# rrwick/Autocycler

Hardware: NVIDIA H100
Metric: input-assembly Mbp/sec through compress->unitig GFA (higher is better)
Workload: dtype u64

## Files before the change

### autocycler_b200/csrc/pipeline.cu

```cuda
#include "pipeline.h"

#include <algorithm>
#include <cmath>
#include <vector>

unsigned long long g_ac_kernel_launches = 0;

#define AC_NONE32 0xFFFFFFFFu
#define AC_CHUNK 32
#define AC_MINCHUNK 128
#define AC_MAX_RANKS 16
#define AC_BOUND_STRIPES 64
#ifndef AC_INSERT_CTAS
#define AC_INSERT_CTAS 2
#endif

struct TableView {
    Slot* slots;
    uint64_t cap;
    const uint64_t* packed;
    const SeqInfo* seqs;
    uint32_t n_seqs;
    uint32_t* count_big;
    uint32_t gb;
// ... 531 lines not shown
};

struct RunAssignBody {
    const uint64_t* run_start; const uint32_t* run_len; const uint32_t* run_uk; const uint8_t* run_dir;
    const uint32_t* uid_rep; const uint32_t* rep_idx; const uint32_t* run_hs; const uint32_t* run_ts; TableView t;
    uint32_t* run_unitig; DeviceUnitig* unitigs; uint32_t* slot_unitig;
    AC_D void operator()(uint64_t r) const {
        const uint32_t rep = uid_rep[run_uk[r]];
        const uint32_t j = rep_idx[rep];
        run_unitig[r] = (j << 1) | (run_dir[r] == run_dir[rep] ? 1u : 0u);
        if (rep == (uint32_t)r) {
            const uint32_t hs = run_hs[r], ts = run_ts[r];
            DeviceUnitig u;
            u.start = run_start[r]; u.len = run_len[r]; u.depth = table_depth(t, hs); u.flip = 0; u.min_d = 0;
            u.head_slot = hs; u.tail_slot = ts;
            for (int w = 0; w < AC_MAX_W; ++w) u.min_w[w] = 0;
            unitigs[j] = u;
            slot_unitig[hs] = j; slot_unitig[ts] = j;
        }
    }
};

struct ClaimedCountBody { const uint32_t* bits; uint64_t n_words; uint32_t* cnt; AC_D void operator()(uint64_t w) const { cnt[w] = w < n_words ? ac_popc(bits[w]) : 0u; } };
template <int W> struct ClaimedListBody {
    const uint32_t* bits; const uint32_t* off; const uint32_t* pos_slot; uint32_t* list;
    TableView t; KParams p; const uint8_t* interior; uint64_t* filter; uint64_t n_fwords;
    AC_D void operator()(uint64_t g) const {
        const uint32_t m = bits[g >> 5], b = (uint32_t)g & 31u;
        if (!((m >> b) & 1u)) return;
        list[off[g >> 5] + ac_popc(m & ((1u << b) - 1u))] = pos_slot[g];
        if (filter) {
            const Key<W> f = window_key<W>(t, g, !interior[g >> 5], p);
            ext_add_kmer<W>(filter, n_fwords, f, key_rc(f, p), p);
        }
    }
};
struct ExportScatterBody {
    TableView t; const uint32_t* occupied; SlotRec* out;
    AC_D void operator()(uint64_t x) const { const uint64_t i = occupied[x]; SlotRec r; r.slot = t.slots[i]; r.count = table_depth(t, i); r.pad = 0; out[x] = r; }
};
template <int W> struct MergeBody {
    TableView t; KParams p; const SlotRec* in; uint32_t* pos_slot; unsigned long long* counters; uint32_t* claimed_bits;
    AC_D void operator()(uint64_t i) const {
        const SlotRec r = in[i];
        const uint64_t g = slot_gpos(r.slot, t.gb);
        const bool dotted = slot_dotted(r.slot, t.gb);
        const uint32_t flags = slot_flags(r.slot);
        const Key<W> fwd = window_key<W>(t, g, dotted, p);
        const Key<W> rc = key_rc(fwd, p);
        const uint64_t h = key_hash(key_is_canonical(fwd, p) ? fwd : rc);
        const uint32_t tag = make_tag(dotted, h, t.gb);
        const Slot mine = make_slot(g, tag, t.count_big ? 0u : r.count, flags, t.gb);
        if (!t.count_big && r.count >= t.alarm) counters[3] = 1;
        uint64_t slot = table_home(t, h);
        for (uint32_t probes = 0;; ++probes) {
            if (probes > 8192) { counters[2] = 1; return; }
            Slot e = ac_ld_cg(&t.slots[slot]);
            if (e == AC_EMPTY_SLOT) {
                e = ac_atomic_cas(&t.slots[slot], (Slot)AC_EMPTY_SLOT, mine);
                if (e == AC_EMPTY_SLOT) { if (t.count_big) ac_atomic_add(&t.count_big[slot], r.count); if (dotted) ac_atomic_add(&counters[1], 1ull); ac_atomic_or(&claimed_bits[g >> 5], 1u << (g & 31u)); break; }
            }
            if (slot_tag(e, t.gb) == tag) {
                const Key<W> rep = window_key<W>(t, slot_gpos(e, t.gb), dotted, p);
                if (key_eq(rep, fwd) || key_eq(rep, rc)) { slot_add_occurrence(t, slot, e, g, r.count, flags, true, counters); break; }
            }
            if (++slot == t.cap) slot = 0;
        }
        pos_slot[g] = (uint32_t)slot;
    }
};

struct ChunkCountBody {
    const DeviceUnitig* unitigs; uint32_t* nchunks;
    AC_D void operator()(uint64_t j) const { nchunks[j] = (unitigs[j].len + AC_MINCHUNK - 1) / AC_MINCHUNK; }
};

template <int W> struct MinPartial { Key<W> key; uint32_t from_rc; };

template <int W> struct ChunkMinBody {
    const uint64_t* packed; const SeqInfo* seqs; uint32_t n_seqs; KParams p;
    const DeviceUnitig* unitigs; uint32_t n_unitigs; const uint32_t* chunk_off; MinPartial<W>* partial;
    AC_D void operator()(uint64_t c) const {
        uint32_t lo = 0, hi = n_unitigs;
        while (hi - lo > 1) { uint32_t mid = (lo + hi) >> 1; if (chunk_off[mid] <= c) lo = mid; else hi = mid; }
        const DeviceUnitig u = unitigs[lo];
        const uint64_t first = (c - chunk_off[lo]) * AC_MINCHUNK;
        const uint64_t n = (u.len - first < AC_MINCHUNK) ? u.len - first : AC_MINCHUNK;
        uint64_t g = u.start + first;
        const SeqInfo s = seqs[find_seq(seqs, n_seqs, g)];
        uint64_t fs = g - s.start;
        Key<W> fwd, rc, best = Key<W>(); bool rolling = false, have = false; uint32_t best_rc = 0;
        for (uint64_t t = 0; t < n; ++t, ++g, ++fs) {
            const int32_t d = window_dots(s, fs, p.k);
            if (d != 0) { fwd = fetch_codes<W>(packed, g, p); fwd.d = d; rc = key_rc(fwd, p); rolling = false; }
            else if (!rolling) { fwd = fetch_codes<W>(packed, g, p); rc = key_rc(fwd, p); rolling = true; }
            else { const uint64_t code = packed_base(packed, g + p.k - 1); key_push_right(fwd, code, p); key_push_left(rc, 3 - code, p); }
            if (!have || key_less5(fwd, best)) { best = fwd; best_rc = 0; have = true; }
            if (key_less5(rc, best)) { best = rc; best_rc = 1; }
        }
        MinPartial<W> out; out.key = best; out.from_rc = best_rc;
        partial[c] = out;
    }
};

template <int W> struct UnitigMinBody {
    const uint32_t* chunk_off; const MinPartial<W>* partial; DeviceUnitig* unitigs;
    AC_D void operator()(uint64_t j) const {
        const uint32_t c0 = chunk_off[j], c1 = chunk_off[j + 1];
        MinPartial<W> best = partial[c0];
        for (uint32_t c = c0 + 1; c < c1; ++c) { const MinPartial<W> q = partial[c]; if (key_less5(q.key, best.key)) best = q; }
        DeviceUnitig u = unitigs[j];
        u.flip = best.from_rc; u.min_d = best.key.d;
        for (int w = 0; w < W; ++w) u.min_w[w] = best.key.w[w];
        unitigs[j] = u;
    }
};

template <int W> struct LinkBody {
    TableView t; KParams p; bool any_dotted;
    const DeviceUnitig* unitigs; const uint32_t* pos_slot; const uint32_t* slot_unitig;
    uint32_t* link_count; uint32_t* links;
    AC_D void operator()(uint64_t i) const {
        const uint32_t j = (uint32_t)(i >> 1), e = (uint32_t)(i & 1);
        const DeviceUnitig u = unitigs[j];
        Key<W> tail, tail_rc;
        if (e == 0) {
            const uint64_t g = u.start + u.len - 1;
            tail = fetch_codes<W>(t.packed, g, p);
            const SeqInfo s = t.seqs[find_seq(t.seqs, t.n_seqs, g)];
            tail.d = window_dots(s, g - s.start, p.k);
            tail_rc = key_rc(tail, p);
        } else {
            const uint64_t g = u.start;
            tail_rc = fetch_codes<W>(t.packed, g, p);
            const SeqInfo s = t.seqs[find_seq(t.seqs, t.n_seqs, g)];
            tail_rc.d = window_dots(s, g - s.start, p.k);
            tail = key_rc(tail_rc, p);
        }
        uint32_t n = 0;
        for_each_successor<W>(tail, tail_rc, any_dotted, p, [&](const Key<W>& a, const Key<W>& arc) {
            const uint32_t s2 = table_find<W>(t, a, arc, p);
            if (s2 == AC_NONE32) return;
            const uint32_t j2 = slot_unitig[s2];
            const DeviceUnitig v = unitigs[j2];
            const bool a_canon = key_is_canonical(a, p);
            const bool head_fwd = v.head_slot == s2 && ((packed_base(t.packed, v.start + p.h) < 2) == a_canon);
            if (n < AC_MAX_LINKS) links[i * AC_MAX_LINKS + n] = (j2 << 1) | (head_fwd ? 0u : 1u);
            ++n;
        });
        link_count[i] = n;
    }
};

struct alignas(16) SortRec { uint64_t a, b; uint32_t c, d, id, pad; };
struct SeedLess {
    const DeviceUnitig* unitigs; int W;
    typedef SortRec Key;
    AC_D Key load(uint32_t id) const {
        const DeviceUnitig& x = unitigs[id];
        Key k; k.id = id; k.pad = 0; k.a = x.min_w[0]; k.b = W > 1 ? x.min_w[1] : 0; k.c = x.min_d > 0 ? (uint32_t)x.min_d : 0u; k.d = x.min_d < 0 ? (uint32_t)-x.min_d : 0u;
        return k;
    }
    AC_D bool less_keys(const Key& x, const Key& y, uint32_t ia, uint32_t ib) const {
        if (x.c != y.c) return x.c > y.c;
        if (x.a != y.a) return x.a < y.a;
        if (x.b != y.b) return x.b < y.b;
        if (W > 2) return (*this)(ia, ib);
        return x.d > y.d;
    }
    AC_D bool operator()(uint32_t a, uint32_t b) const {
        const DeviceUnitig& x = unitigs[a]; const DeviceUnitig& y = unitigs[b];
        const int lx = x.min_d > 0 ? x.min_d : 0, ly = y.min_d > 0 ? y.min_d : 0;
        if (lx != ly) return lx > ly;
        for (int w = 0; w < W; ++w) if (x.min_w[w] != y.min_w[w]) return x.min_w[w] < y.min_w[w];
        const int tx = x.min_d < 0 ? -x.min_d : 0, ty = y.min_d < 0 ? -y.min_d : 0;
        return tx > ty;
    }
};
#define AC_SORT_LEAF 8
#define AC_SORT_WAYS 8
template <class Less> struct MergeWaysBody {
    Less less; uint32_t n, width, steps; const SortRec* in; SortRec* out; uint32_t* idx_out;
    AC_D void operator()(uint64_t i) const {
        const SortRec me = in[i];
        const uint64_t run = i / width, group = run / AC_SORT_WAYS, group_start = group * AC_SORT_WAYS * (uint64_t)width;
        uint32_t lo[AC_SORT_WAYS], hi[AC_SORT_WAYS];
#pragma unroll
        for (int s = 0; s < AC_SORT_WAYS; ++s) {
            const uint64_t first = group_start + (uint64_t)s * width, last = first + width;
            lo[s] = (uint32_t)(first < n ? first : n); hi[s] = (uint32_t)(last < n ? last : n);
            if (group * AC_SORT_WAYS + s == run) hi[s] = lo[s];
        }
        for (uint32_t step = 0; step < steps; ++step) {
#pragma unroll
            for (int s = 0; s < AC_SORT_WAYS; ++s) {
                if (lo[s] < hi[s]) {
                    const uint32_t mid = (lo[s] + hi[s]) >> 1;
                    const SortRec x = in[mid];
                    const bool earlier = group * AC_SORT_WAYS + s < run;
                    const bool before = earlier ? !less.less_keys(me, x, me.id, x.id) : less.less_keys(x, me, x.id, me.id);
                    if (before) lo[s] = mid + 1; else hi[s] = mid;
                }
            }
        }
        uint64_t pos = group_start + (i - run * width);
#pragma unroll
        for (int s = 0; s < AC_SORT_WAYS; ++s) {
            const uint64_t first = group_start + (uint64_t)s * width;
            if (group * AC_SORT_WAYS + s != run && first < n) pos += lo[s] - (uint32_t)first;
        }
        out[pos] = me; idx_out[pos] = me.id;
    }
};

#ifndef AC_EMULATE
#define AC_SORT_TILE 2048
#else
#define AC_SORT_TILE 16
#endif
#ifndef AC_EMULATE
template <class Less> __global__ void __launch_bounds__(1024) ac_tile_sort_kernel(const Less less, uint32_t n, uint32_t* __restrict__ idx, SortRec* __restrict__ recs) {
    extern __shared__ __align__(16) unsigned char tile_smem[];
    SortRec* keys = reinterpret_cast<SortRec*>(tile_smem);
    uint16_t* buf0 = reinterpret_cast<uint16_t*>(tile_smem + AC_SORT_TILE * sizeof(SortRec));
    uint16_t* buf1 = buf0 + AC_SORT_TILE;
    const uint32_t base = blockIdx.x * AC_SORT_TILE, count = n - base < AC_SORT_TILE ? n - base : AC_SORT_TILE;
    for (uint32_t i = threadIdx.x; i < count; i += blockDim.x) { SortRec r = less.load(base + i); r.id = base + i; r.pad = 0; keys[i] = r; }
    __syncthreads();
    auto before = [&](uint32_t x, uint32_t y) { return less.less_keys(keys[x], keys[y], base + x, base + y); };
    if (threadIdx.x < AC_SORT_TILE / AC_SORT_LEAF) {
        const uint32_t a = threadIdx.x * AC_SORT_LEAF, b = a + AC_SORT_LEAF < count ? a + AC_SORT_LEAF : count;
        uint16_t v[AC_SORT_LEAF];
        for (uint32_t x = a; x < b; ++x) {
            uint32_t y = x - a;
            while (y > 0 && before(x, v[y - 1])) { v[y] = v[y - 1]; --y; }
            v[y] = (uint16_t)x;
        }
        for (uint32_t x = a; x < b; ++x) buf0[x] = v[x - a];
    }
    __syncthreads();
    uint16_t* in = buf0; uint16_t* out = buf1;
    for (uint32_t width = AC_SORT_LEAF; width < count; width *= 2) {
        for (uint32_t i = threadIdx.x; i < count; i += blockDim.x) {
            const uint32_t me = in[i];
            const uint32_t run = i / width, pair_start = (run & ~1u) * width, run_start = run * width;
            const bool left = !(run & 1u);
            uint32_t lo, hi;
            if (left) { lo = run_start + width; hi = lo + width; } else { lo = pair_start; hi = run_start; }
            if (lo > count) lo = count;
            if (hi > count) hi = count;
            const uint32_t first = lo;
            while (lo < hi) { const uint32_t mid = (lo + hi) >> 1; const bool bf = left ? before(in[mid], me) : !before(me, in[mid]); if (bf) lo = mid + 1; else hi = mid; }
            out[pair_start + (i - run_start) + (lo - first)] = (uint16_t)me;
        }
        __syncthreads();
        uint16_t* t = in; in = out; out = t;
    }
    for (uint32_t i = threadIdx.x; i < count; i += blockDim.x) { const SortRec r = keys[in[i]]; recs[base + i] = r; idx[base + i] = r.id; }
}
#endif
template <class Less> struct TileSortBody {
    Less less; uint32_t n; uint32_t* idx; SortRec* recs;
    AC_D void operator()(uint64_t c) const {
        const uint32_t a = (uint32_t)c * AC_SORT_TILE, b = a + AC_SORT_TILE < n ? a + AC_SORT_TILE : n;
        for (uint32_t x = a; x < b; ++x) {
            uint32_t y = x;
            while (y > a && less(x, idx[y - 1])) { idx[y] = idx[y - 1]; --y; }
            idx[y] = x;
        }
        for (uint32_t x = a; x < b; ++x) { SortRec r = less.load(idx[x]); r.id = idx[x]; r.pad = 0; recs[x] = r; }
    }
};
template <class Less> static uint32_t* sort_indices(AcStream* stream, const Less& less, uint32_t n, uint32_t* a, uint32_t* b, SortRec* ra, SortRec* rb) {
    if (n == 0) return a;
    const uint64_t tiles = ((uint64_t)n + AC_SORT_TILE - 1) / AC_SORT_TILE;
#ifndef AC_EMULATE
    const size_t smem = AC_SORT_TILE * (sizeof(SortRec) + 2 * sizeof(uint16_t));
    ac_launch_kernel("tile_sort", stream, ac_tile_sort_kernel<Less>, (unsigned)tiles, 1024, smem, less, n, a, ra);
#else
    ac_launch("tile_sort", stream, TileSortBody<Less>{less, n, a, ra}, tiles);
#endif
    for (uint64_t width = AC_SORT_TILE; width < n; width *= AC_SORT_WAYS) {
        uint32_t steps = 1; while ((1ull << steps) <= width) ++steps;
        ac_launch("merge_pass", stream, MergeWaysBody<Less>{less, n, (uint32_t)width, steps, ra, rb, b}, n);
        std::swap(a, b); std::swap(ra, rb);
    }
    return a;
}

struct NumberKeyBody {
    const UnitigRec* rec; const char* arena; uint64_t* prefix;
    AC_D void operator()(uint64_t s) const {
        const unsigned char* q = (const unsigned char*)(arena + rec[s].seq_off);
        const uint32_t m = rec[s].len < 8 ? rec[s].len : 8;
        uint64_t v = 0;
        for (uint32_t i = 0; i < m; ++i) v |= (uint64_t)q[i] << (56 - 8 * i);
        prefix[s] = v;
    }
};
struct InversePermBody { const uint32_t* order; uint32_t* pos; AC_D void operator()(uint64_t n) const { pos[order[n]] = (uint32_t)n; } };
struct NumberLess {
    const UnitigRec* rec; const uint32_t* depth; const char* arena; const uint64_t* prefix;
    const uint32_t* pos;
    typedef SortRec Key;
    AC_D Key load(uint32_t id) const { Key k; k.id = id; k.pad = 0; k.a = prefix[id]; k.b = pos ? pos[id] : id; k.c = rec[id].len; k.d = depth[id]; return k; }
    AC_D bool less_keys(const Key& x, const Key& y, uint32_t ia, uint32_t ib) const {
        if (x.c != y.c) return x.c > y.c;
        if (x.a != y.a) return x.a < y.a;
        if (x.c > 8) return (*this)(ia, ib);
        if (x.d != y.d) return x.d > y.d;
        return x.b < y.b;
    }
    AC_D bool operator()(uint32_t a, uint32_t b) const {
        const uint32_t la = rec[a].len, lb = rec[b].len;
        if (la != lb) return la > lb;
        if (prefix[a] != prefix[b]) return prefix[a] < prefix[b];
        const char* x = arena + rec[a].seq_off; const char* y = arena + rec[b].seq_off;
        for (uint32_t i = 8; i < la; ++i) if (x[i] != y[i]) return (unsigned char)x[i] < (unsigned char)y[i];
        if (depth[a] != depth[b]) return depth[a] > depth[b];
        return pos ? pos[a] < pos[b] : a < b;
    }
};


struct SeedGatherBody {
    const uint32_t* perm; const DeviceUnitig* unitigs; uint32_t n;
    uint32_t* rank; uint32_t* len; uint32_t* depth; uint32_t* need; uint32_t* min_fpos; uint32_t* min_rpos;
    AC_D void operator()(uint64_t s) const {
        if (s == n) { need[s] = 0; return; }
        const uint32_t j = perm[s];
        const DeviceUnitig& u = unitigs[j];
        rank[j] = (uint32_t)s; len[s] = u.len; depth[s] = u.depth; need[s] = u.len + 2 * AC_SEQ_SLACK;
        min_fpos[s] = 0xFFFFFFFFu; min_rpos[s] = 0xFFFFFFFFu;
    }
};
struct SeqOffBody { const uint32_t* need_off; uint64_t* seq_off; AC_D void operator()(uint64_t s) const { seq_off[s] = (uint64_t)need_off[s] + AC_SEQ_SLACK; } };

struct EmitSeqBody {
    const uint64_t* packed; uint32_t h; const DeviceUnitig* unitigs; uint32_t n_unitigs; const uint32_t* chunk_off;
    const uint32_t* rank; const uint64_t* seq_off; char* arena;
    AC_D void operator()(uint64_t c) const {
        uint32_t lo = 0, hi = n_unitigs;
        while (hi - lo > 1) { uint32_t mid = (lo + hi) >> 1; if (chunk_off[mid] <= c) lo = mid; else hi = mid; }
        const DeviceUnitig u = unitigs[lo];
        const uint64_t first = (c - chunk_off[lo]) * AC_MINCHUNK;
        const uint64_t n = (u.len - first < AC_MINCHUNK) ? u.len - first : AC_MINCHUNK;
        char* dst = arena + seq_off[rank[lo]];
        const uint64_t g0 = u.start + h + first;
        if (!u.flip) for (uint64_t t = 0; t < n; ++t) dst[first + t] = "ACGT"[packed_base(packed, g0 + t)];
        else for (uint64_t t = 0; t < n; ++t) dst[u.len - 1 - (first + t)] = "TGCA"[packed_base(packed, g0 + t)];
    }
};

AC_D UStrand seed_strand(uint32_t dev_strand, const uint32_t* rank, const DeviceUnitig* unitigs) {
    const uint32_t j = dev_strand >> 1;
    return (rank[j] << 1) | ((dev_strand & 1u) ^ (unitigs[j].flip & 1u));
}

struct LinkCountBody {
    const uint32_t* link_count; const uint32_t* rank; const DeviceUnitig* unitigs; uint32_t n_strands; uint32_t* cnt;
    AC_D void operator()(uint64_t i) const {
        if (i == n_strands) { cnt[i] = 0; return; }
        cnt[seed_strand((uint32_t)i, rank, unitigs)] = link_count[i];
    }
};

struct LinkOrderBody {
    const uint32_t* link_count; const uint32_t* links; const uint32_t* rank; const DeviceUnitig* unitigs;
    const uint32_t* next_off; UStrand* next; uint32_t* prev_cnt; uint32_t* hairpins;
    AC_D static uint64_t order_key(UStrand from, UStrand t) {
        const uint32_t a = from >> 1, b = t >> 1; const bool trev = t & 1;
        uint32_t phase;
        if (!(from & 1)) phase = trev ? 1 : 0;
        else phase = trev ? (b < a ? 0 : (b == a ? 1 : 3)) : 2;
        return ((uint64_t)phase << 32) | b;
    }
    AC_D void operator()(uint64_t i) const {
        const UStrand from = seed_strand((uint32_t)i, rank, unitigs);
        const uint32_t n = link_count[i];
        UStrand t[AC_MAX_LINKS];
        for (uint32_t x = 0; x < n && x < AC_MAX_LINKS; ++x) t[x] = seed_strand(links[i * AC_MAX_LINKS + x], rank, unitigs);
        for (uint32_t x = 1; x < n; ++x) {
            const UStrand v = t[x]; const uint64_t kv = order_key(from, v); uint32_t y = x;
            while (y > 0 && order_key(from, t[y - 1]) > kv) { t[y] = t[y - 1]; --y; }
            t[y] = v;
        }
        UStrand* out = next + next_off[from];
        for (uint32_t x = 0; x < n; ++x) { out[x] = t[x]; ac_atomic_add(&prev_cnt[t[x]], 1u); if (t[x] == (from ^ 1u)) ac_atomic_add(hairpins, 1u); }
    }
};
struct PrevFillBody {
    const uint32_t* next_off; const UStrand* next; const uint32_t* prev_off; uint32_t* cursor; UStrand* prev;
    AC_D void operator()(uint64_t from) const {
        for (uint32_t x = next_off[from]; x < next_off[from + 1]; ++x) { const UStrand t = next[x]; prev[prev_off[t] + ac_atomic_add(&cursor[t], 1u)] = (UStrand)from; }
    }
};
struct PrevSortBody {
    const uint32_t* prev_off; UStrand* prev;
    AC_D void operator()(uint64_t s) const {
        UStrand* p = prev + prev_off[s]; const uint32_t n = prev_off[s + 1] - prev_off[s];
        for (uint32_t x = 1; x < n; ++x) { const UStrand v = p[x]; uint32_t y = x; while (y > 0 && p[y - 1] > v) { p[y] = p[y - 1]; --y; } p[y] = v; }
    }
};

struct PathBody {
    const SeqInfo* seqs; uint32_t n_seqs; const uint64_t* run_start; const uint32_t* run_len; const uint32_t* run_unitig;
    const uint32_t* rank; const DeviceUnitig* unitigs; UStrand* path; uint32_t* min_fpos; uint32_t* min_rpos;
    AC_D void operator()(uint64_t x) const {
        const uint32_t dev = run_unitig[x] >> 1, same = run_unitig[x] & 1;
        const uint32_t s = rank[dev];
        const bool plus = (same ^ (unitigs[dev].flip & 1u)) != 0;
        path[x] = (s << 1) | (plus ? 0u : 1u);
        const uint64_t g = run_start[x];
        const SeqInfo q = seqs[find_seq(seqs, n_seqs, g)];
        const uint32_t fs = (uint32_t)(g - q.start), mirrored = q.len - fs - run_len[x];
        ac_atomic_min(&min_fpos[s], plus ? fs : mirrored);
        ac_atomic_min(&min_rpos[s], plus ? mirrored : fs);
    }
};
struct PackRecBody {
    const uint64_t* seq_off; const uint32_t* len; const uint32_t* min_fpos; const uint32_t* min_rpos; UnitigRec* rec;
    AC_D void operator()(uint64_t s) const {
        UnitigRec r; r.seq_off = seq_off[s]; r.len = len[s]; r.min_fpos = min_fpos[s]; r.min_rpos = min_rpos[s];
        r.room_before = AC_SEQ_SLACK; r.room_after = AC_SEQ_SLACK; r.flags = 0;
        rec[s] = r;
    }
};
struct FixedSeedBody {
    const uint64_t* path_off; const UStrand* path; uint8_t* fixed_start; uint8_t* fixed_end;
    AC_D void operator()(uint64_t i) const {
        if (path_off[i + 1] == path_off[i]) return;
        const UStrand first = path[path_off[i]], last = path[path_off[i + 1] - 1];
        if (!(first & 1u)) fixed_start[first >> 1] = 1; else fixed_end[first >> 1] = 1;
        if (!(last & 1u)) fixed_end[last >> 1] = 1; else fixed_start[last >> 1] = 1;
    }
};
struct FixedSpreadBody {
    const uint8_t* seed_start; const uint8_t* seed_end; const uint32_t* next_off; const UStrand* next; const uint32_t* prev_off; const UStrand* prev;
    uint8_t* fixed_start; uint8_t* fixed_end;
    AC_D void operator()(uint64_t u) const {
        const uint32_t s = (uint32_t)u << 1;
        if (seed_start[u]) for (uint32_t x = prev_off[s]; x < prev_off[s + 1]; ++x) { const UStrand up = prev[x]; if (!(up & 1u)) fixed_end[up >> 1] = 1; else fixed_start[up >> 1] = 1; }
        if (seed_end[u]) for (uint32_t x = next_off[s]; x < next_off[s + 1]; ++x) { const UStrand down = next[x]; if (!(down & 1u)) fixed_start[down >> 1] = 1; else fixed_end[down >> 1] = 1; }
    }
};
struct CandidateView {
    const uint32_t* order; const uint32_t* next_off; const UStrand* next; const uint32_t* prev_off; const UStrand* prev;
    const uint8_t* fixed_start; const uint8_t* fixed_end;
    AC_D bool eligible(uint32_t idx, uint32_t side) const {
        const UStrand self = idx << 1;
        const uint32_t* off = side == 0 ? prev_off : next_off; const UStrand* lst = side == 0 ? prev : next;
        const uint32_t* back_off = side == 0 ? next_off : prev_off; const UStrand* back = side == 0 ? next : prev;
        const uint32_t gn = off[self + 1] - off[self];
        if (gn < 2 || (side == 0 ? fixed_start[idx] : fixed_end[idx])) return false;
        for (uint32_t a = 0; a < gn; ++a) {
            const UStrand p = lst[off[self] + a];
            if (back_off[p + 1] - back_off[p] != 1 || back[back_off[p]] != self || (p >> 1) == idx) return false;
            const bool rev = p & 1u;
            if (side == 0 ? ((!rev && fixed_end[p >> 1]) || (rev && fixed_start[p >> 1])) : ((!rev && fixed_start[p >> 1]) || (rev && fixed_end[p >> 1]))) return false;
        }
        return true;
    }
};
struct CandidateFlagBody {
    CandidateView v; uint32_t n; uint32_t* flag;
    AC_D void operator()(uint64_t x) const {
        if (x == 2ull * n) { flag[x] = 0; return; }
        flag[x] = v.eligible(v.order[x >> 1], (uint32_t)(x & 1)) ? 1u : 0u;
    }
};
struct CandidateFillBody {
// ... 883 lines not shown
    }
    any_dotted = n_dotted != 0;
    const TableView tv = table_view();

    flags8.ensure(cap);
    n_slots_used = list_claimed<W>(true);
    const AdjacencyBody<W> adj{tv, p, any_dotted, occ_list.as<uint32_t>(), flags8.as<uint8_t>(), ext_filter.as<uint64_t>(), n_fwords};
    if (is_multi && exp_valid && exp_n + 64 < n_slots_used) {
        const uint64_t n_cw = (total + 31) / 32, n_adj = exp_n + 64;
        if (getenv("AC_HOST_PROFILE")) fprintf(stderr, "[device] adjacency flags for this rank's own k-mers: at most %llu of %llu\n", (unsigned long long)n_adj, (unsigned long long)n_slots_used);
        ac_launch("adjacency", &stream, AdjacencyOwnBody<W>{adj, claimed_cnt.as<uint32_t>(), g_begin >> 5, std::min<uint64_t>((g_end + 31) >> 5, n_cw)}, n_adj);
    } else ac_launch("adjacency", &stream, adj, n_slots_used);
    mark(ADJACENCY_END);

    const uint64_t n_bwords = (total + 31) / 32;
    bmask.ensure(n_bwords * sizeof(uint32_t)); bcount.ensure(n_bwords * sizeof(uint32_t)); boff.ensure(n_bwords * sizeof(uint32_t));
    ac_launch("boundaries", &stream, BoundaryBody{packed.as<uint64_t>(), seqs.as<SeqInfo>(), n_seqs, p.h, g_begin, g_end, pos_slot.as<uint32_t>(),
                                                  flags8.as<uint8_t>(), interior8.as<uint8_t>(), bmask.as<uint32_t>(), bcount.as<uint32_t>()}, n_bwords * 32);
    n_runs = scan(&stream, bcount.as<uint32_t>(), boff.as<uint32_t>(), n_bwords);
    mark(BOUNDARIES_END);
    run_start.ensure(n_runs * sizeof(uint64_t)); run_len.ensure(n_runs * 4); run_hs.ensure(n_runs * 4); run_ts.ensure(n_runs * 4);
    ac_launch("run_scatter", &stream, RunScatterBody{bmask.as<uint32_t>(), boff.as<uint32_t>(), run_start.as<uint64_t>()}, n_bwords);
    ac_launch("run_ends", &stream, RunEndsLocalBody{seqs.as<SeqInfo>(), n_seqs, run_start.as<uint64_t>(), n_runs, pos_slot.as<uint32_t>(),
                                                    run_len.as<uint32_t>(), run_hs.as<uint32_t>(), run_ts.as<uint32_t>()}, n_runs);
    n_own_runs = n_runs;
    stage = Stage::RUNS;
}

void DevicePipeline::export_runs(void* dst, uint64_t cap_records) {
    Impl& m = *impl; m.make_current();
    m.require(Stage::RUNS, "runs_local must precede export_runs");
    if (cap_records < m.n_runs) throw std::runtime_error("run buffer too small");
    ac_launch("run_export", &m.stream, RunExportBody{m.run_start.as<uint64_t>(), m.run_len.as<uint32_t>(), m.run_hs.as<uint32_t>(), m.run_ts.as<uint32_t>(),
                                                     m.slots.as<Slot>(), slot_gpos_bits(m.total), (RunRec*)dst}, m.n_runs);
    ac_sync(&m.stream);
}

void DevicePipeline::import_runs(const void* dev_ptr, uint64_t n) {
    Impl& m = *impl; m.make_current();
    m.require(Stage::RUNS, "runs_local must precede import_runs");
    m.n_runs = n;
    m.run_start.ensure(n * sizeof(uint64_t)); m.run_len.ensure(n * 4); m.run_hs.ensure(n * 4); m.run_ts.ensure(n * 4);
    RunImportBody body{(const RunRec*)dev_ptr, m.pos_slot.as<uint32_t>(), m.run_start.as<uint64_t>(), m.run_len.as<uint32_t>(), m.run_hs.as<uint32_t>(), m.run_ts.as<uint32_t>(), 0, {0}, {nullptr}};
    ac_launch("run_import", &m.stream, body, n);
}

void DevicePipeline::import_runs_from(const void* const* ptrs, const uint64_t* counts, uint32_t n_ranks) {
    Impl& m = *impl; m.make_current();
    m.require(Stage::RUNS, "runs_local must precede import_runs");
    if (n_ranks == 0 || n_ranks > AC_MAX_RANKS) throw std::runtime_error("import_runs: bad rank count");
    RunImportBody body{nullptr, m.pos_slot.as<uint32_t>(), nullptr, nullptr, nullptr, nullptr, n_ranks, {0}, {nullptr}};
    for (uint32_t q = 0; q < n_ranks; ++q) { body.first[q + 1] = body.first[q] + counts[q]; body.src[q] = (const RunRec*)ptrs[q]; }
    const uint64_t n = m.n_runs = body.first[n_ranks];
    m.run_start.ensure(n * sizeof(uint64_t)); m.run_len.ensure(n * 4); m.run_hs.ensure(n * 4); m.run_ts.ensure(n * 4);
    body.run_start = m.run_start.as<uint64_t>(); body.run_len = m.run_len.as<uint32_t>(); body.run_hs = m.run_hs.as<uint32_t>(); body.run_ts = m.run_ts.as<uint32_t>();
    ac_launch("run_import", &m.stream, body, n);
}

void DevicePipeline::finish(PipelineResult& out, bool keep_positions, bool fused, bool split_paths) {
    Impl& m = *impl; m.make_current(); const int W = m.W;
    if (split_paths && !fused) throw std::runtime_error("split path lines need the fused finish");
    AC_DISPATCH_W(m.unitigs_w, out)
    m.host_arrays();
    m.paths();
    m.work_list();
    if (fused && m.R.n_cands > 0) m.simplify();
    m.mark(SIMPLIFY_END);
    if (fused) {
        m.renumber();
        if (m.U < 100000000u) m.gfa(split_paths);
    }
    m.mark(GFA_END);
    m.results(out, keep_positions, fused);
}

template <int W> void DevicePipeline::Impl::unitigs_w(PipelineResult& out) {
    require(Stage::RUNS, "runs_local must precede finish");
    const KParams p = make_kparams(k, W);
    const TableView tv = table_view();
    out = PipelineResult();
    out.W = W; out.capacity = cap; out.n_slots_used = n_slots_used; out.n_dotted = n_dotted;
    R = Pending();
    mark(FINISH_BEGIN);
    run_uk.ensure(n_runs * 4); run_dir.ensure(n_runs);
    is_rep.ensure(n_runs * 4); rep_idx.ensure(n_runs * 4); run_unitig.ensure(n_runs * 4);
    uid_rep.ensure(cap * 4); slot_unitig.ensure(cap * 4);
    ac_memset(uid_rep.p, 0xFF, cap * 4, &stream);
    ac_launch("run_key", &stream, RunKeyBody{packed.as<uint64_t>(), p.h, run_start.as<uint64_t>(), run_hs.as<uint32_t>(), run_ts.as<uint32_t>(),
                                             run_uk.as<uint32_t>(), run_dir.as<uint8_t>(), uid_rep.as<uint32_t>()}, n_runs);
    ac_launch("rep_flag", &stream, RepFlagBody{run_uk.as<uint32_t>(), uid_rep.as<uint32_t>(), is_rep.as<uint32_t>()}, n_runs);
    U = scan(&stream, is_rep.as<uint32_t>(), rep_idx.as<uint32_t>(), n_runs);
    unitigs.ensure((size_t)U * sizeof(DeviceUnitig));
    ac_launch("run_assign", &stream, RunAssignBody{run_start.as<uint64_t>(), run_len.as<uint32_t>(), run_uk.as<uint32_t>(), run_dir.as<uint8_t>(),
                                                   uid_rep.as<uint32_t>(), rep_idx.as<uint32_t>(), run_hs.as<uint32_t>(), run_ts.as<uint32_t>(), tv,
                                                   run_unitig.as<uint32_t>(), unitigs.as<DeviceUnitig>(), slot_unitig.as<uint32_t>()}, n_runs);
    mark(UNITIGS_END);

    nchunks.ensure(((size_t)U + 1) * 4); chunk_off.ensure(((size_t)U + 1) * 4);
    ac_launch("chunk_count", &stream, ChunkCountBody{unitigs.as<DeviceUnitig>(), nchunks.as<uint32_t>()}, U);
    ac_memset(nchunks.as<uint32_t>() + U, 0, 4, &stream);
    n_chunks = scan(&stream, nchunks.as<uint32_t>(), chunk_off.as<uint32_t>(), (uint64_t)U + 1);
    partial.ensure((size_t)n_chunks * sizeof(MinPartial<W>));
    ac_launch("chunk_min", &stream, ChunkMinBody<W>{packed.as<uint64_t>(), seqs.as<SeqInfo>(), n_seqs, p, unitigs.as<DeviceUnitig>(), U,
                                                    chunk_off.as<uint32_t>(), partial.as<MinPartial<W>>()}, n_chunks);
    ac_launch("unitig_min", &stream, UnitigMinBody<W>{chunk_off.as<uint32_t>(), partial.as<MinPartial<W>>(), unitigs.as<DeviceUnitig>()}, U);
    mark(SEEDS_END);

    link_count.ensure((size_t)U * 2 * 4); links.ensure((size_t)U * 2 * AC_MAX_LINKS * 4);
    ac_launch("links", &stream, LinkBody<W>{tv, p, any_dotted, unitigs.as<DeviceUnitig>(), pos_slot.as<uint32_t>(), slot_unitig.as<uint32_t>(),
                                            link_count.as<uint32_t>(), links.as<uint32_t>()}, (uint64_t)U * 2);
    mark(LINKS_END);
}

void DevicePipeline::Impl::host_arrays() {
    sort_a.ensure((size_t)U * 4); sort_b.ensure((size_t)U * 4); sort_ra.ensure((size_t)U * sizeof(SortRec)); sort_rb.ensure((size_t)U * sizeof(SortRec));
    const SeedLess seed_less{unitigs.as<DeviceUnitig>(), W};
    const uint32_t* perm = sort_indices(&stream, seed_less, U, sort_a.as<uint32_t>(), sort_b.as<uint32_t>(), sort_ra.as<SortRec>(), sort_rb.as<SortRec>());
    mark(SEED_SORT_END);
    rank.ensure((size_t)U * 4); d_len.ensure((size_t)U * 4); d_depth.ensure((size_t)U * 4); need.ensure(((size_t)U + 1) * 4);
    d_seq_off.ensure((size_t)U * 8); d_min_fpos.ensure((size_t)U * 4); d_min_rpos.ensure((size_t)U * 4);
    ac_launch("seed_gather", &stream, SeedGatherBody{perm, unitigs.as<DeviceUnitig>(), U, rank.as<uint32_t>(), d_len.as<uint32_t>(), d_depth.as<uint32_t>(),
                                                     need.as<uint32_t>(), d_min_fpos.as<uint32_t>(), d_min_rpos.as<uint32_t>()}, (uint64_t)U + 1);
    if (n_windows + (uint64_t)U * 2 * AC_SEQ_SLACK >= 0xFFFFFFF0ull) throw std::runtime_error("unitig sequence arena would exceed 4 GB");
    const uint64_t arena_bytes = scan(&stream, need.as<uint32_t>(), need.as<uint32_t>(), (uint64_t)U + 1);
    ac_launch("seq_off", &stream, SeqOffBody{need.as<uint32_t>(), d_seq_off.as<uint64_t>()}, U);
    d_arena.ensure(arena_bytes);
    ac_launch("emit_seq", &stream, EmitSeqBody{packed.as<uint64_t>(), make_kparams(k, W).h, unitigs.as<DeviceUnitig>(), U, chunk_off.as<uint32_t>(), rank.as<uint32_t>(),
                                               d_seq_off.as<uint64_t>(), d_arena.as<char>()}, n_chunks);
    R.arena_final = arena_bytes; R.arena_src = &d_arena;
    const uint32_t n_strands = 2 * U;
    strand_cnt.ensure(((size_t)n_strands + 1) * 4); d_next_off.ensure(((size_t)n_strands + 1) * 4);
    prev_cnt.ensure(((size_t)n_strands + 1) * 4); d_prev_off.ensure(((size_t)n_strands + 1) * 4);
    ac_launch("link_count", &stream, LinkCountBody{link_count.as<uint32_t>(), rank.as<uint32_t>(), unitigs.as<DeviceUnitig>(), n_strands, strand_cnt.as<uint32_t>()},
              (uint64_t)n_strands + 1);
    const uint64_t n_links = R.n_links = scan(&stream, strand_cnt.as<uint32_t>(), d_next_off.as<uint32_t>(), (uint64_t)n_strands + 1);
    d_next.ensure(n_links * 4); d_prev.ensure(n_links * 4);
    ac_memset(prev_cnt.p, 0, ((size_t)n_strands + 1) * 4, &stream);
    d_small.ensure(64); ac_memset(d_small.p, 0, 64, &stream);
    ac_launch("link_order", &stream, LinkOrderBody{link_count.as<uint32_t>(), links.as<uint32_t>(), rank.as<uint32_t>(), unitigs.as<DeviceUnitig>(),
                                                   d_next_off.as<uint32_t>(), d_next.as<UStrand>(), prev_cnt.as<uint32_t>(), d_small.as<uint32_t>()}, n_strands);
    scan(&stream, prev_cnt.as<uint32_t>(), d_prev_off.as<uint32_t>(), (uint64_t)n_strands + 1, false);
    ac_memset(prev_cnt.p, 0, ((size_t)n_strands + 1) * 4, &stream);
    ac_launch("prev_fill", &stream, PrevFillBody{d_next_off.as<uint32_t>(), d_next.as<UStrand>(), d_prev_off.as<uint32_t>(), prev_cnt.as<uint32_t>(), d_prev.as<UStrand>()}, n_strands);
    ac_launch("prev_sort", &stream, PrevSortBody{d_prev_off.as<uint32_t>(), d_prev.as<UStrand>()}, n_strands);
}

void DevicePipeline::Impl::paths() {
    d_path.ensure(n_runs * 4); d_path_off.ensure(((size_t)n_seqs + 1) * 8);
    ac_launch("path", &stream, PathBody{seqs.as<SeqInfo>(), n_seqs, run_start.as<uint64_t>(), run_len.as<uint32_t>(), run_unitig.as<uint32_t>(), rank.as<uint32_t>(),
                                        unitigs.as<DeviceUnitig>(), d_path.as<UStrand>(), d_min_fpos.as<uint32_t>(), d_min_rpos.as<uint32_t>()}, n_runs);
    d_rec.ensure((size_t)U * sizeof(UnitigRec));
    ac_launch("pack_rec", &stream, PackRecBody{d_seq_off.as<uint64_t>(), d_len.as<uint32_t>(), d_min_fpos.as<uint32_t>(), d_min_rpos.as<uint32_t>(), d_rec.as<UnitigRec>()}, U);
    ac_launch("path_off", &stream, PathOffBody{seqs.as<SeqInfo>(), n_seqs, run_start.as<uint64_t>(), n_runs, d_path_off.as<uint64_t>()}, (uint64_t)n_seqs + 1);
    num_prefix.ensure((size_t)U * 8);
    ac_launch("number_key", &stream, NumberKeyBody{d_rec.as<UnitigRec>(), d_arena.as<char>(), num_prefix.as<uint64_t>()}, U);
    const NumberLess number_less{d_rec.as<UnitigRec>(), d_depth.as<uint32_t>(), d_arena.as<char>(), num_prefix.as<uint64_t>(), nullptr};
    R.order_built = sort_indices(&stream, number_less, U, sort_a.as<uint32_t>(), sort_b.as<uint32_t>(), sort_ra.as<SortRec>(), sort_rb.as<SortRec>());
}

void DevicePipeline::Impl::work_list() {
    d_fixed.ensure((size_t)U * 4); ac_memset(d_fixed.p, 0, (size_t)U * 4, &stream);
    uint8_t* seed_start = d_fixed.as<uint8_t>(); uint8_t* seed_end = seed_start + U; uint8_t* fix_start = R.fix_start = seed_end + U; uint8_t* fix_end = fix_start + U;
    ac_launch("fixed_seed", &stream, FixedSeedBody{d_path_off.as<uint64_t>(), d_path.as<UStrand>(), seed_start, seed_end}, n_seqs);
    ac_copy_dd(fix_start, seed_start, (size_t)U * 2, &stream);
    ac_launch("fixed_spread", &stream, FixedSpreadBody{seed_start, seed_end, d_next_off.as<uint32_t>(), d_next.as<UStrand>(), d_prev_off.as<uint32_t>(), d_prev.as<UStrand>(),
                                                       fix_start, fix_end}, U);
    const CandidateView cview{R.order_built, d_next_off.as<uint32_t>(), d_next.as<UStrand>(), d_prev_off.as<uint32_t>(), d_prev.as<UStrand>(), fix_start, fix_end};
    cand_flag.ensure((2 * (size_t)U + 1) * 4); cand_index.ensure((2 * (size_t)U + 1) * 4);
    ac_launch("candidate_flag", &stream, CandidateFlagBody{cview, U, cand_flag.as<uint32_t>()}, 2ull * U + 1);
    const uint64_t n_cands = R.n_cands = scan(&stream, cand_flag.as<uint32_t>(), cand_index.as<uint32_t>(), 2ull * U + 1);
    d_cands.ensure((n_cands + 1) * sizeof(ExpandCandidate)); d_cand_at.ensure(2 * (size_t)U * 4 + 4); d_deps.ensure((size_t)U * sizeof(ExpandDeps) + 4); d_spec.ensure((n_cands + 1) * 4);
    ac_launch("candidate_fill", &stream, CandidateFillBody{cview, cand_flag.as<uint32_t>(), cand_index.as<uint32_t>(), d_cands.as<ExpandCandidate>(), d_cand_at.as<int32_t>()}, 2ull * U);
    ac_launch("dependents", &stream, DependentsBody{d_next_off.as<uint32_t>(), d_next.as<UStrand>(), d_prev_off.as<uint32_t>(), d_prev.as<UStrand>(), d_cand_at.as<int32_t>(),
                                                    d_deps.as<ExpandDeps>()}, U);
    ac_launch("common_length", &stream, CommonLengthBody{d_cands.as<ExpandCandidate>(), d_rec.as<UnitigRec>(), d_arena.as<char>(), d_spec.as<uint32_t>()}, n_cands);
    mark(WORK_LIST_END);
}

void DevicePipeline::Impl::simplify() {
    const uint64_t n_cands = R.n_cands, arena_bytes = R.arena_final;
    d_pred.ensure(n_cands * 7 * 4); d_level.ensure(n_cands * 4); d_flagmax.ensure(32); d_counters64.ensure((AC_PASS_WORDS + 8) * 8);
    d_dirty.ensure(((n_cands + 63) / 64) * 8 + 8); d_exhausted.ensure(n_cands + 8);
    unsigned long long* c64 = d_counters64.as<unsigned long long>();
    unsigned long long* res = c64 + AC_PASS_WORDS;
    ac_launch("level_pred", &stream, LevelPredBody{d_cands.as<ExpandCandidate>(), d_deps.as<ExpandDeps>(), d_pred.as<int32_t>()}, n_cands);
    ac_memset(d_level.p, 0, n_cands * 4, &stream); ac_memset(d_flagmax.p, 0, 32, &stream);
    ac_launch_coop("levels", &stream, LevelsCoopBody{d_pred.as<int32_t>(), d_level.as<uint32_t>(), d_flagmax.as<uint32_t>(), n_cands}, n_cands, 1024);
    ac_memset(d_counters64.p, 0, (AC_PASS_WORDS + 8) * 8, &stream);
    const RelocBoundBody bound_body{d_cands.as<ExpandCandidate>(), d_rec.as<UnitigRec>(), d_cand_at.as<int32_t>(), c64 + AC_PASS_SET(1) + 1};
    ac_launch("reloc_bound", &stream, bound_body, n_cands);
    uint32_t fm[8]; unsigned long long h64[AC_PASS_WORDS + 8];
    ac_d2h(fm, d_flagmax.p, 32, &stream); ac_d2h(h64, c64, sizeof h64, &stream); ac_sync(&stream);
    if (fm[4]) throw std::runtime_error("candidate levels did not settle");
    unsigned long long bound = 0; for (int x = 0; x < AC_BOUND_STRIPES; ++x) bound += h64[AC_PASS_SET(1) + 1 + x];
    if (arena_bytes + bound >= 0xFFFFFFF0ull) throw std::runtime_error("unitig sequence arena would exceed 4 GB");
    d_arena2.ensure(arena_bytes + 2 * bound + 64);
    ac_copy_dd(d_arena2.p, d_arena.p, arena_bytes, &stream);
    const unsigned long long start = arena_bytes;
    ac_h2d(c64, &start, 8, &stream);
    ac_memset(c64 + AC_PASS_SET(1), 0, AC_PASS_SET_WORDS * 8, &stream);
    ac_memset(d_dirty.p, 0, ((n_cands + 63) / 64) * 8 + 8, &stream); ac_memset(d_exhausted.p, 0, n_cands + 8, &stream);
    static const bool always_grow = getenv("AC_DEVICE_TIGHT_ARENA") != nullptr;
    uint32_t next_set = 0, next_due = 0; uint64_t passes = 0;
    const uint32_t due_stride = fm[3] + 2;
    d_due.ensure((size_t)3 * due_stride * 4); ac_memset(d_due.p, 0, (size_t)3 * due_stride * 4, &stream);
    for (bool first = true;; first = false) {
        const ApplyLevelBody apply{d_cands.as<ExpandCandidate>(), d_deps.as<ExpandDeps>(), d_level.as<uint32_t>(), 0, d_spec.as<uint32_t>(),
                                   d_rec.as<UnitigRec>(), d_arena2.as<char>(), c64, c64, d_dirty.as<uint64_t>(), d_exhausted.as<uint8_t>(), first, c64 + AC_PASS_REMOVED};
        const uint64_t room = always_grow ? 0 : d_arena2.cap;
        ac_launch_coop("simplify", &stream, SimplifyCoopBody{apply, bound_body, n_cands, d_flagmax.as<uint32_t>() + 3, c64, res, room, next_set, first,
                                                             d_due.as<uint32_t>(), due_stride, next_due}, n_cands, 64);
        ac_d2h(h64, c64, sizeof h64, &stream); ac_sync(&stream);
        const unsigned long long* r = h64 + AC_PASS_WORDS;
        R.arena_final = h64[0]; R.bases_removed = h64[AC_PASS_REMOVED]; R.any_moved = r[1] != 0;
        passes += r[2]; next_set = (uint32_t)r[5]; next_due = (uint32_t)r[7];
        if (getenv("AC_HOST_PROFILE")) fprintf(stderr, "[device] expand_repeats launch: %llu passes (%llu so far), %u levels, %llu candidates, %llu left on the work list, last pass moved %llu bases\n",
                                               r[2], (unsigned long long)passes, fm[3], (unsigned long long)n_cands, r[4], r[0]);
        if (r[0] == 0) break;
        if (passes > 1000000) throw std::runtime_error("repeat expansion did not settle");
        bound = r[3];
        if (R.arena_final + bound >= 0xFFFFFFF0ull) throw std::runtime_error("unitig sequence arena would exceed 4 GB");
        d_arena3.ensure(std::max<size_t>((R.arena_final + bound) * 2 + 64, d_arena3.cap + (always_grow ? 64 : 0)));
        ac_copy_dd(d_arena3.p, d_arena2.p, R.arena_final, &stream); ac_sync(&stream);
        std::swap(d_arena2.p, d_arena3.p); std::swap(d_arena2.cap, d_arena3.cap);
    }
    R.arena_src = &d_arena2;
}

void DevicePipeline::Impl::renumber() {
    if (!R.any_moved) { R.final_order = R.order_built; return; }
    d_pos.ensure((size_t)U * 4); sort_c.ensure((size_t)U * 4); sort_d.ensure((size_t)U * 4);
    ac_launch("inverse_perm", &stream, InversePermBody{R.order_built, d_pos.as<uint32_t>()}, U);
    ac_launch("number_key", &stream, NumberKeyBody{d_rec.as<UnitigRec>(), R.arena_src->as<char>(), num_prefix.as<uint64_t>()}, U);
    const NumberLess final_less{d_rec.as<UnitigRec>(), d_depth.as<uint32_t>(), R.arena_src->as<char>(), num_prefix.as<uint64_t>(), d_pos.as<uint32_t>()};
    R.final_order = sort_indices(&stream, final_less, U, sort_c.as<uint32_t>(), sort_d.as<uint32_t>(), sort_ra.as<SortRec>(), sort_rb.as<SortRec>());
}

void DevicePipeline::Impl::gfa(bool split_paths) {
    d_pos2.ensure((size_t)U * 4);
    ac_launch("inverse_perm", &stream, InversePermBody{R.final_order, d_pos2.as<uint32_t>()}, U);
    const GfaView gv{R.final_order, d_pos2.as<uint32_t>(), d_rec.as<UnitigRec>(), R.arena_src->as<char>(), d_depth.as<uint32_t>(), d_next_off.as<uint32_t>(), d_next.as<UStrand>()};
    gfa_s_size.ensure(((size_t)U + 1) * 4); gfa_l_size.ensure(((size_t)U + 1) * 4); gfa_pieces.ensure(((size_t)U + 1) * 4);
    const uint64_t steps = split_paths ? 0 : n_runs;
    d_last.ensure(steps + 8); gfa_p_size.ensure((steps + 1) * 4);
    ac_launch("gfa_size", &stream, GfaSizeBody{gv, U, gfa_s_size.as<uint32_t>(), gfa_l_size.as<uint32_t>()}, (uint64_t)U + 1);
    ac_launch("gfa_chunk_count", &stream, GfaChunkCountBody{gv, U, gfa_pieces.as<uint32_t>()}, (uint64_t)U + 1);
    d_totals.ensure(64); ac_memset(d_totals.p, 0, 64, &stream);
    if (!split_paths) {
        ac_memset(d_last.p, 0, steps + 8, &stream);
        ac_launch("path_last", &stream, PathLastBody{d_path_off.as<uint64_t>(), d_last.as<uint8_t>()}, n_seqs);
        ac_launch("path_size", &stream, PathSizeBody{d_path.as<UStrand>(), d_pos2.as<uint32_t>(), d_last.as<uint8_t>(), steps, gfa_p_size.as<uint32_t>()}, steps + 1);
        scan.keep_total(&stream, gfa_p_size.as<uint32_t>(), steps + 1, d_totals.as<uint32_t>() + 3);
    }
    scan.keep_total(&stream, gfa_s_size.as<uint32_t>(), (uint64_t)U + 1, d_totals.as<uint32_t>() + 0);
    scan.keep_total(&stream, gfa_l_size.as<uint32_t>(), (uint64_t)U + 1, d_totals.as<uint32_t>() + 1);
    scan.keep_total(&stream, gfa_pieces.as<uint32_t>(), (uint64_t)U + 1, d_totals.as<uint32_t>() + 2);
    uint32_t tot[4];
    ac_d2h(tot, d_totals.p, 16, &stream); ac_sync(&stream);
    const uint64_t s_bytes = tot[0], l_bytes = tot[1], n_pieces = tot[2], p_list_bytes = tot[3];
    char head[64]; const uint64_t head_bytes = (uint64_t)snprintf(head, sizeof head, "H\tVN:Z:1.0\tKM:i:%u\n", k);
    if (path_wrap_total == 0 && n_seqs) throw std::runtime_error("set_path_line_texts() must precede a build that renders the GFA");
    const uint64_t p_bytes = split_paths ? 0 : p_list_bytes + path_wrap_total;
    R.gfa_bytes = head_bytes + s_bytes + l_bytes + p_bytes;
    d_text.ensure(R.gfa_bytes + 64);
    char* text = d_text.as<char>();
    ac_h2d(text, head, head_bytes, &stream);
    ac_launch("gfa_segment", &stream, GfaSegmentBody{gv, gfa_s_size.as<uint32_t>(), text + head_bytes}, U);
    ac_launch("gfa_sequence", &stream, GfaSequenceBody{gv, U, gfa_pieces.as<uint32_t>(), gfa_s_size.as<uint32_t>(), text + head_bytes}, 32 * n_pieces);
    h_text.ensure(R.gfa_bytes + 64);
    copy_text_after_rendering(head_bytes + s_bytes);
    ac_launch("gfa_link", &stream, GfaLinkBody{gv, gfa_l_size.as<uint32_t>(), text + head_bytes + s_bytes}, U);
    copy_text_after_rendering(head_bytes + s_bytes + l_bytes);
    const PathLineView pv{d_path_off.as<uint64_t>(), n_seqs, gfa_p_size.as<uint32_t>(), d_wrap_off.as<uint64_t>(), d_pre_len.as<uint32_t>(), d_suf_len.as<uint32_t>(),
                          d_blob.as<char>(), d_blob_off.as<uint64_t>(), 0};
    char* p_text = text + head_bytes + s_bytes + l_bytes;
    if (!split_paths) {
        ac_launch("path_text", &stream, PathTextFullBody{d_path.as<UStrand>(), d_pos2.as<uint32_t>(), d_last.as<uint8_t>(), pv, p_text}, steps);
        ac_launch("path_wrap", &stream, PathWrapBody{pv, p_text}, 64ull * n_seqs);
    }
    R.paths_split = split_paths;
    R.gfa_on_device = true;
}

void DevicePipeline::Impl::results(PipelineResult& out, bool keep_positions, bool fused) {
    if (before_results && *before_results) (*before_results)();
    out.fused = fused; out.graph_fetched = false;
    if (fused && !R.gfa_on_device) throw std::runtime_error("fused build: the device GFA writer did not run");
    uint64_t d2h = 0;
    if (R.gfa_on_device) {
        copy_text_after_rendering(R.gfa_bytes);
        ac_record(&text_copied, &copy_stream); ac_wait(&stream, &text_copied);
        d2h += R.gfa_bytes;
    }
    uint32_t small[16];
    ac_d2h(small, d_small.p, 64, &stream); ac_sync(&stream); d2h += 64;
    out.links_single = (R.n_links - small[0]) / 2 + small[0];
    out.length_before = n_slots_used;
    out.length_after = n_slots_used - R.bases_removed;
    out.gfa_text = R.gfa_on_device ? h_text.as<char>() : nullptr; out.gfa_bytes = R.gfa_on_device ? R.gfa_bytes : 0;
    out.n_unitigs = U; out.n_runs = n_runs; out.n_seqs = n_seqs; out.n_links = R.n_links;
    out.h2d_bytes = uploaded_bytes + (uint64_t)n_seqs * sizeof(SeqInfo);
    out.d2h_bytes = d2h;
    if (!fused) pull_graph(out, keep_positions);
    else { mark(ALL_BUT_ARENA); mark(RESULTS_END); arena_pending = true; }
}

void DevicePipeline::Impl::pull_graph(PipelineResult& out, bool keep_positions) {
// ... 170 lines not shown
```

Baseline: 5484.

## Use packed 2-bit sequence keys and head prefixes to avoid deep comparator fallbacks in sorts

Unitig numbering keys now pack up to 64 bases as 2-bit codes in two words instead of 8 raw bytes. The comparators no longer fall back to indexed global-memory comparisons during merges; ties beyond the packed key are resolved afterwards by a separate tie-run insertion-sort pass. The tile sort also caches a 64-bit head key in shared memory for fast first comparisons, and the merge pass is launched with an occupancy hint. This adds a kernel, more shared memory and prefix storage, and relies on the tie-run pass being correct for long equal-prefix runs.

After: 5551, median of 6. 1.01x the previous value.

```diff
diff --git a/autocycler_b200/csrc/pipeline.cu b/autocycler_b200/csrc/pipeline.cu
--- a/autocycler_b200/csrc/pipeline.cu
+++ b/autocycler_b200/csrc/pipeline.cu
@@ -707,22 +707,25 @@
     }
 };
 
-struct alignas(16) SortRec { uint64_t a, b; uint32_t c, d, id, pad; };
+struct alignas(16) SortRec { uint64_t a, b; uint32_t c, d, e, id; };
 struct SeedLess {
     const DeviceUnitig* unitigs; int W;
     typedef SortRec Key;
     AC_D Key load(uint32_t id) const {
         const DeviceUnitig& x = unitigs[id];
-        Key k; k.id = id; k.pad = 0; k.a = x.min_w[0]; k.b = W > 1 ? x.min_w[1] : 0; k.c = x.min_d > 0 ? (uint32_t)x.min_d : 0u; k.d = x.min_d < 0 ? (uint32_t)-x.min_d : 0u;
+        Key k; k.id = id; k.e = 0; k.a = x.min_w[0]; k.b = W > 1 ? x.min_w[1] : 0; k.c = x.min_d > 0 ? (uint32_t)x.min_d : 0u; k.d = x.min_d < 0 ? (uint32_t)-x.min_d : 0u;
         return k;
     }
-    AC_D bool less_keys(const Key& x, const Key& y, uint32_t ia, uint32_t ib) const {
+    AC_D bool less_keys(const Key& x, const Key& y) const {
         if (x.c != y.c) return x.c > y.c;
         if (x.a != y.a) return x.a < y.a;
         if (x.b != y.b) return x.b < y.b;
-        if (W > 2) return (*this)(ia, ib);
-        return x.d > y.d;
-    }
+        if (x.d != y.d) return x.d > y.d;
+        return x.id < y.id;
+    }
+    AC_D uint64_t head(const Key& x) const { return ((uint64_t)(0xFFFFu - x.c) << 48) | (x.a >> 16); }
+    bool may_tie() const { return W > 2; }
+    AC_D bool tied(const Key& x, const Key& y) const { return W > 2 && x.c == y.c && x.a == y.a && x.b == y.b; }
     AC_D bool operator()(uint32_t a, uint32_t b) const {
         const DeviceUnitig& x = unitigs[a]; const DeviceUnitig& y = unitigs[b];
         const int lx = x.min_d > 0 ? x.min_d : 0, ly = y.min_d > 0 ? y.min_d : 0;
@@ -753,7 +756,7 @@
                     const uint32_t mid = (lo[s] + hi[s]) >> 1;
                     const SortRec x = in[mid];
                     const bool earlier = group * AC_SORT_WAYS + s < run;
-                    const bool before = earlier ? !less.less_keys(me, x, me.id, x.id) : less.less_keys(x, me, x.id, me.id);
+                    const bool before = earlier ? !less.less_keys(me, x) : less.less_keys(x, me);
                     if (before) lo[s] = mid + 1; else hi[s] = mid;
                 }
             }
@@ -777,12 +780,13 @@
 template <class Less> __global__ void __launch_bounds__(1024) ac_tile_sort_kernel(const Less less, uint32_t n, uint32_t* __restrict__ idx, SortRec* __restrict__ recs) {
     extern __shared__ __align__(16) unsigned char tile_smem[];
     SortRec* keys = reinterpret_cast<SortRec*>(tile_smem);
-    uint16_t* buf0 = reinterpret_cast<uint16_t*>(tile_smem + AC_SORT_TILE * sizeof(SortRec));
+    uint64_t* heads = reinterpret_cast<uint64_t*>(tile_smem + AC_SORT_TILE * sizeof(SortRec));
+    uint16_t* buf0 = reinterpret_cast<uint16_t*>(heads + AC_SORT_TILE);
     uint16_t* buf1 = buf0 + AC_SORT_TILE;
     const uint32_t base = blockIdx.x * AC_SORT_TILE, count = n - base < AC_SORT_TILE ? n - base : AC_SORT_TILE;
-    for (uint32_t i = threadIdx.x; i < count; i += blockDim.x) { SortRec r = less.load(base + i); r.id = base + i; r.pad = 0; keys[i] = r; }
+    for (uint32_t i = threadIdx.x; i < count; i += blockDim.x) { const SortRec r = less.load(base + i); keys[i] = r; heads[i] = less.head(r); }
     __syncthreads();
-    auto before = [&](uint32_t x, uint32_t y) { return less.less_keys(keys[x], keys[y], base + x, base + y); };
+    auto before = [&](uint32_t x, uint32_t y) { const uint64_t hx = heads[x], hy = heads[y]; return hx != hy ? hx < hy : less.less_keys(keys[x], keys[y]); };
     if (threadIdx.x < AC_SORT_TILE / AC_SORT_LEAF) {
         const uint32_t a = threadIdx.x * AC_SORT_LEAF, b = a + AC_SORT_LEAF < count ? a + AC_SORT_LEAF : count;
         uint16_t v[AC_SORT_LEAF];
@@ -819,38 +823,63 @@
     AC_D void operator()(uint64_t c) const {
         const uint32_t a = (uint32_t)c * AC_SORT_TILE, b = a + AC_SORT_TILE < n ? a + AC_SORT_TILE : n;
         for (uint32_t x = a; x < b; ++x) {
+            const SortRec r = less.load(x);
             uint32_t y = x;
-            while (y > a && less(x, idx[y - 1])) { idx[y] = idx[y - 1]; --y; }
-            idx[y] = x;
-        }
-        for (uint32_t x = a; x < b; ++x) { SortRec r = less.load(idx[x]); r.id = idx[x]; r.pad = 0; recs[x] = r; }
+            while (y > a && (less.head(r) != less.head(recs[y - 1]) ? less.head(r) < less.head(recs[y - 1]) : less.less_keys(r, recs[y - 1]))) { recs[y] = recs[y - 1]; --y; }
+            recs[y] = r;
+        }
+        for (uint32_t x = a; x < b; ++x) idx[x] = recs[x].id;
+    }
+};
+template <class Less> struct TieRunBody {
+    Less less; uint32_t n; const SortRec* recs; uint32_t* idx;
+    AC_D void operator()(uint64_t i) const {
+        if (i > 0 && less.tied(recs[i - 1], recs[i])) return;
+        uint64_t end = i + 1;
+        while (end < n && less.tied(recs[end - 1], recs[end])) ++end;
+        for (uint64_t x = i + 1; x < end; ++x) {
+            const uint32_t v = idx[x];
+            uint64_t y = x;
+            while (y > i && less(v, idx[y - 1])) { idx[y] = idx[y - 1]; --y; }
+            idx[y] = v;
+        }
     }
 };
 template <class Less> static uint32_t* sort_indices(AcStream* stream, const Less& less, uint32_t n, uint32_t* a, uint32_t* b, SortRec* ra, SortRec* rb) {
     if (n == 0) return a;
     const uint64_t tiles = ((uint64_t)n + AC_SORT_TILE - 1) / AC_SORT_TILE;
 #ifndef AC_EMULATE
-    const size_t smem = AC_SORT_TILE * (sizeof(SortRec) + 2 * sizeof(uint16_t));
+    const size_t smem = AC_SORT_TILE * (sizeof(SortRec) + sizeof(uint64_t) + 2 * sizeof(uint16_t));
     ac_launch_kernel("tile_sort", stream, ac_tile_sort_kernel<Less>, (unsigned)tiles, 1024, smem, less, n, a, ra);
 #else
     ac_launch("tile_sort", stream, TileSortBody<Less>{less, n, a, ra}, tiles);
 #endif
     for (uint64_t width = AC_SORT_TILE; width < n; width *= AC_SORT_WAYS) {
         uint32_t steps = 1; while ((1ull << steps) <= width) ++steps;
-        ac_launch("merge_pass", stream, MergeWaysBody<Less>{less, n, (uint32_t)width, steps, ra, rb, b}, n);
+        ac_launch_occ<4>("merge_pass", stream, MergeWaysBody<Less>{less, n, (uint32_t)width, steps, ra, rb, b}, n);
         std::swap(a, b); std::swap(ra, rb);
     }
+    if (less.may_tie()) ac_launch("tie_runs", stream, TieRunBody<Less>{less, n, ra, a}, n);
     return a;
 }
 
+#define AC_NUMBER_KEY_BASES 64
 struct NumberKeyBody {
     const UnitigRec* rec; const char* arena; uint64_t* prefix;
     AC_D void operator()(uint64_t s) const {
-        const unsigned char* q = (const unsigned char*)(arena + rec[s].seq_off);
-        const uint32_t m = rec[s].len < 8 ? rec[s].len : 8;
-        uint64_t v = 0;
-        for (uint32_t i = 0; i < m; ++i) v |= (uint64_t)q[i] << (56 - 8 * i);
-        prefix[s] = v;
+        const uint64_t off = rec[s].seq_off;
+        const uint32_t m = rec[s].len < AC_NUMBER_KEY_BASES ? rec[s].len : AC_NUMBER_KEY_BASES;
+        uint64_t w0 = 0, w1 = 0;
+        uint32_t i = 0;
+        for (uint64_t a = off & ~7ull; i < m; a += 8) {
+            const uint64_t word = *reinterpret_cast<const uint64_t*>(arena + a);
+            for (uint32_t b = a < off ? (uint32_t)(off - a) : 0u; b < 8 && i < m; ++b, ++i) {
+                const uint32_t c = (uint32_t)(word >> (8 * b)) & 0xFFu;
+                const uint64_t code = c < 'C' ? 0 : c < 'G' ? 1 : c < 'T' ? 2 : 3;
+                if (i < 32) w0 |= code << (62 - 2 * i); else w1 |= code << (62 - 2 * (i - 32));
+            }
+        }
+        prefix[2 * s] = w0; prefix[2 * s + 1] = w1;
     }
 };
 struct InversePermBody { const uint32_t* order; uint32_t* pos; AC_D void operator()(uint64_t n) const { pos[order[n]] = (uint32_t)n; } };
@@ -858,20 +887,22 @@
     const UnitigRec* rec; const uint32_t* depth; const char* arena; const uint64_t* prefix;
     const uint32_t* pos;
     typedef SortRec Key;
-    AC_D Key load(uint32_t id) const { Key k; k.id = id; k.pad = 0; k.a = prefix[id]; k.b = pos ? pos[id] : id; k.c = rec[id].len; k.d = depth[id]; return k; }
-    AC_D bool less_keys(const Key& x, const Key& y, uint32_t ia, uint32_t ib) const {
+    AC_D Key load(uint32_t id) const { Key k; k.id = id; k.a = prefix[2 * id]; k.b = prefix[2 * id + 1]; k.c = rec[id].len; k.d = depth[id]; k.e = pos ? pos[id] : id; return k; }
+    AC_D bool less_keys(const Key& x, const Key& y) const {
         if (x.c != y.c) return x.c > y.c;
         if (x.a != y.a) return x.a < y.a;
-        if (x.c > 8) return (*this)(ia, ib);
+        if (x.b != y.b) return x.b < y.b;
         if (x.d != y.d) return x.d > y.d;
-        return x.b < y.b;
-    }
+        return x.e < y.e;
+    }
+    AC_D uint64_t head(const Key& x) const { return ((uint64_t)~x.c << 32) | (x.a >> 32); }
+    bool may_tie() const { return true; }
+    AC_D bool tied(const Key& x, const Key& y) const { return x.c == y.c && x.c > AC_NUMBER_KEY_BASES && x.a == y.a && x.b == y.b; }
     AC_D bool operator()(uint32_t a, uint32_t b) const {
         const uint32_t la = rec[a].len, lb = rec[b].len;
         if (la != lb) return la > lb;
-        if (prefix[a] != prefix[b]) return prefix[a] < prefix[b];
         const char* x = arena + rec[a].seq_off; const char* y = arena + rec[b].seq_off;
-        for (uint32_t i = 8; i < la; ++i) if (x[i] != y[i]) return (unsigned char)x[i] < (unsigned char)y[i];
+        for (uint32_t i = 0; i < la; ++i) if (x[i] != y[i]) return (unsigned char)x[i] < (unsigned char)y[i];
         if (depth[a] != depth[b]) return depth[a] > depth[b];
         return pos ? pos[a] < pos[b] : a < b;
     }
@@ -2061,7 +2092,7 @@
     d_rec.ensure((size_t)U * sizeof(UnitigRec));
     ac_launch("pack_rec", &stream, PackRecBody{d_seq_off.as<uint64_t>(), d_len.as<uint32_t>(), d_min_fpos.as<uint32_t>(), d_min_rpos.as<uint32_t>(), d_rec.as<UnitigRec>()}, U);
     ac_launch("path_off", &stream, PathOffBody{seqs.as<SeqInfo>(), n_seqs, run_start.as<uint64_t>(), n_runs, d_path_off.as<uint64_t>()}, (uint64_t)n_seqs + 1);
-    num_prefix.ensure((size_t)U * 8);
+    num_prefix.ensure((size_t)U * 16);
     ac_launch("number_key", &stream, NumberKeyBody{d_rec.as<UnitigRec>(), d_arena.as<char>(), num_prefix.as<uint64_t>()}, U);
     const NumberLess number_less{d_rec.as<UnitigRec>(), d_depth.as<uint32_t>(), d_arena.as<char>(), num_prefix.as<uint64_t>(), nullptr};
     R.order_built = sort_indices(&stream, number_less, U, sort_a.as<uint32_t>(), sort_b.as<uint32_t>(), sort_ra.as<SortRec>(), sort_rb.as<SortRec>());
```
